# lanxinger/spz

Hardware: AMD Instinct MI355X
Metric: Gaussians/s encode+decode (SH3, 10M pts) (higher is better)
Workload: dtype f32

## Files before the change

### spz_amd/csrc/spz_abi.hip

```cpp
#include <hip/hip_runtime.h>

#include <cmath>
#include <cstdint>
#include <algorithm>
#include <cstdlib>
#include <cstring>
#include <mutex>

#include "spz_amd.h"
#include "spz_common.hpp"
#include "spz_kernel_params.hpp"

namespace spz_amd_detail {
thread_local int g_last_hip_error = 0;

}

namespace {

using namespace spz_amd_detail;

constexpr uint32_t kMagic = 0x5053474eu;

unsigned long long sh_elem_mask_ext(uint32_t sh15, int sh_dim) {
// ... 85 lines not shown
    SPZ_HIP_TRY(hipMalloc(reinterpret_cast<void **>(&d), sizeof(float) * kTableFloats));
    hipError_t e = hipMemcpy(d, g_tables.host, sizeof(float) * kTableFloats, hipMemcpyHostToDevice);
    if (e != hipSuccess) {
      g_last_hip_error = (int)e;
      (void)hipFree(d);
      return SPZ_AMD_ERR_HIP;
    }
    g_tables.dev[device] = d;
  }
  *dev_tables = g_tables.dev[device];
  return SPZ_AMD_OK;
}
}

namespace {

int grid_for(int device, uint32_t total_tiles, uint32_t *grid) {
  uint32_t cap = 0x7fffffffu;
  if (kMaxBlocksPerCU > 0) {
    static int cus[kMaxDevices] = {0};
    if (cus[device] == 0) {
      int n = 0;
      SPZ_HIP_TRY(hipDeviceGetAttribute(&n, hipDeviceAttributeMultiprocessorCount, device));
      cus[device] = (n > 0) ? n : 256;
    }
    cap = (uint32_t)cus[device] * (uint32_t)kMaxBlocksPerCU;
  }
  uint32_t g = total_tiles < cap ? total_tiles : cap;
#if SPZ_XCD_REMAP
  g = ((total_tiles + 7u) / 8u) * 8u;
#endif
  *grid = g > 0 ? g : 1;
  return SPZ_AMD_OK;
}

void add_section(KParams *p, uint32_t tile_units, uint32_t kind, uint8_t *bytes, float *floats,
                 unsigned long long n_elems) {
  if (n_elems == 0) return;
  SecDesc &s = p->sec[p->n_sec++];
  s.bytes = bytes;
  s.floats = floats;
  s.n_elems = n_elems;
  s.n_units = (n_elems + 3) / 4;
  s.tile_begin = p->total_tiles;
  s.tile_skip = 0;
  s.kind = kind;
  p->total_tiles += (uint32_t)((s.n_units + tile_units - 1) / tile_units);
}

void interleave_sections(KParams *p) {
  const uint32_t n = p->n_sec, total = p->total_tiles;
  if (n < 2 || total < 4 * kIlPeriod) return;
  constexpr uint32_t G = SPZ_IL_GROUP;
  uint32_t tiles[SPZ_AMD_NUM_SECTIONS], count[SPZ_AMD_NUM_SECTIONS], used = 0;
  uint32_t big = 0, part_total = 0;
  for (uint32_t k = 0; k < n; ++k) {
    tiles[k] = (k + 1 < n ? p->sec[k + 1].tile_begin : total) - p->sec[k].tile_begin;
    big = tiles[k] > tiles[big] ? k : big;
  }
  auto takes_part = [&](uint32_t k) {
    return !SPZ_IL_ONLY_ROT || k == big || p->sec[k].kind == KIND_ROT_S3 || p->sec[k].kind == KIND_ROT_F3;
  };
  for (uint32_t k = 0; k < n; ++k) part_total += takes_part(k) ? tiles[k] : 0u;
  for (uint32_t k = 0; k < n; ++k) {
    count[k] = takes_part(k) ? (uint32_t)(((unsigned long long)tiles[k] * kIlPeriod + part_total / 2) / part_total) : 0u;
    used += count[k];
  }
  if (used > kIlPeriod && count[big] <= used - kIlPeriod) return;
  count[big] = count[big] + kIlPeriod - used;
  uint32_t reps = 0xffffffffu;
  for (uint32_t k = 0; k < n; ++k) {
    if (count[k]) reps = tiles[k] / (count[k] * G) < reps ? tiles[k] / (count[k] * G) : reps;
  }
  if (reps == 0 || reps == 0xffffffffu) return;
  uint32_t given[SPZ_AMD_NUM_SECTIONS] = {};
  for (uint32_t slot = 0; slot < kIlPeriod; ++slot) {
    uint32_t best = n;
    unsigned long long best_pos = ~0ull;
    for (uint32_t k = 0; k < n; ++k) {
      if (given[k] >= count[k]) continue;
      const unsigned long long pos = (2ull * given[k] + 1ull) * kIlPeriod * 1024ull / (2ull * count[k]);
      if (pos < best_pos) {
        best_pos = pos;
        best = k;
      }
    }
    p->il_sec[slot] = (uint8_t)best;
    p->il_rank[slot] = (uint8_t)given[best];
    ++given[best];
  }
  p->il_tiles = reps * kIlPeriod * G;
  uint32_t begin = p->il_tiles;
  for (uint32_t k = 0; k < n; ++k) {
    p->il_count[k] = (uint8_t)count[k];
    p->sec[k].tile_skip = reps * count[k] * G;
    p->sec[k].tile_begin = begin;
    begin += tiles[k] - reps * count[k] * G;
  }
}

int grid_order_override() {
  const char *e = std::getenv("SPZ_AMD_GRID_ORDER");
  if (e == nullptr) return 0;
  if (std::strcmp(e, "sequential") == 0) return 1;
  if (std::strcmp(e, "interleaved") == 0) return 2;
  return 0;
}

int layout_impl(uint64_t n, int sh_degree, int version, spz_amd_layout *out) {
  const int sd = sh_dim_for_degree(sh_degree);
  if (sd < 0 || version < 1 || version > 3 || out == nullptr) return SPZ_AMD_ERR_INVALID_ARG;
  const uint32_t bpp[SPZ_AMD_NUM_SECTIONS] = {version == 1 ? 6u : 9u, 1u, 3u, 3u, version >= 3 ? 4u : 3u,
                                               (uint32_t)sd * 3u};
  uint64_t off = 16;
  for (int s = 0; s < SPZ_AMD_NUM_SECTIONS; ++s) {
    out->bytes_per_point[s] = bpp[s];
    out->offset[s] = off;
    out->bytes[s] = n * bpp[s];
    off += out->bytes[s];
  }
  out->total_bytes = off;
  return SPZ_AMD_OK;
}

int encode_impl(const spz_amd_cloud_in *cl, uint64_t first, uint64_t count, uint64_t n_total, int sh_degree,
                int antialiased, int from_coord, int version, int write_header, uint8_t *d_stream,
                size_t capacity, void *hip_stream, unsigned section_mask = 0x3fu) {
  if (cl == nullptr || d_stream == nullptr || !valid_coord(from_coord)) return SPZ_AMD_ERR_INVALID_ARG;
  if (version == 1) return SPZ_AMD_ERR_UNSUPPORTED;
  spz_amd_layout lay;
  int rc = layout_impl(n_total, sh_degree, version, &lay);
  if (rc != SPZ_AMD_OK) return rc;
  if (n_total > 0xffffffffull || first > n_total || count > n_total - first) return SPZ_AMD_ERR_INVALID_ARG;
  if (capacity < lay.total_bytes) return SPZ_AMD_ERR_CAPACITY;
  const int sd = sh_dim_for_degree(sh_degree);
  if (count > 0 && (!cl->positions || !cl->scales || !cl->rotations || !cl->alphas || !cl->colors ||
                    (sd > 0 && !cl->sh))) {
    return SPZ_AMD_ERR_INVALID_ARG;
  }
  int device = 0;
  rc = current_device(&device);
  if (rc != SPZ_AMD_OK) return rc;
  KParams p = {};
  rc = ensure_tables(device, &p.tables);
  if (rc != SPZ_AMD_OK) return rc;

  const FlipMasks fm = flip_masks(from_coord, SPZ_AMD_RUB);
  p.flip_p = fm.p;
  p.flip_q = fm.q;
  p.sh_mask_ext = sh_elem_mask_ext(fm.sh15, sd);
  p.sh_d = (uint32_t)sd * 3u;
  p.pos_scale = 0.0f;
  auto frag = [&](int s) { return d_stream + lay.offset[s] + first * lay.bytes_per_point[s]; };
  auto fl = [](const float *q) { return const_cast<float *>(q); };
  auto want = [&](int s) { return ((section_mask >> s) & 1u) != 0u; };
  if (want(SPZ_AMD_SEC_SH)) add_section(&p, EncGeom::kTileUnits, KIND_SH, frag(SPZ_AMD_SEC_SH), fl(cl->sh), count * (uint64_t)sd * 3u);
  if (want(SPZ_AMD_SEC_POSITIONS)) add_section(&p, EncGeom::kTileUnits, KIND_POS24, frag(SPZ_AMD_SEC_POSITIONS), fl(cl->positions), count * 3u);
  if (want(SPZ_AMD_SEC_ROTATIONS)) {
    add_section(&p, EncGeom::kTileUnits, version >= 3 ? KIND_ROT_S3 : KIND_ROT_F3, frag(SPZ_AMD_SEC_ROTATIONS), fl(cl->rotations),
                count * 4u);
  }
  if (want(SPZ_AMD_SEC_SCALES)) add_section(&p, EncGeom::kTileUnits, KIND_SCALE, frag(SPZ_AMD_SEC_SCALES), fl(cl->scales), count * 3u);
  if (want(SPZ_AMD_SEC_COLORS)) add_section(&p, EncGeom::kTileUnits, KIND_COLOR, frag(SPZ_AMD_SEC_COLORS), fl(cl->colors), count * 3u);
  if (want(SPZ_AMD_SEC_ALPHAS)) add_section(&p, EncGeom::kTileUnits, KIND_ALPHA, frag(SPZ_AMD_SEC_ALPHAS), fl(cl->alphas), count);
  if (write_header) {
    p.header_dst = d_stream;
    p.header_words[0] = kMagic;
    p.header_words[1] = (uint32_t)version;
    p.header_words[2] = (uint32_t)n_total;
    p.header_words[3] = (uint32_t)sh_degree | (12u << 8) | ((antialiased ? 1u : 0u) << 16);
  }
  if (p.total_tiles == 0 && !write_header) return SPZ_AMD_OK;
  {
    const int order = grid_order_override();
    if (order == 2 || (order == 0 && (SPZ_ENC_INTERLEAVE == 1 || (SPZ_ENC_INTERLEAVE == 2 && sd == 0)))) interleave_sections(&p);
  }
  uint32_t grid = 1;
  rc = grid_for(device, p.total_tiles, &grid);
  if (rc != SPZ_AMD_OK) return rc;
  hipLaunchKernelGGL(spz_encode_kernel, dim3(grid), dim3(EncGeom::kBlock), 0, static_cast<hipStream_t>(hip_stream), p);
  SPZ_HIP_TRY(hipGetLastError());
  return SPZ_AMD_OK;
}

int check_header_fields(const spz_amd_header *h) {
  if (h == nullptr) return SPZ_AMD_ERR_INVALID_ARG;
  if (h->version < 1 || h->version > 3) return SPZ_AMD_ERR_VERSION;
  if (h->sh_degree > 3) return SPZ_AMD_ERR_SH_DEGREE;
  return SPZ_AMD_OK;
}

int decode_impl(const uint8_t *d_stream, size_t size, const spz_amd_header *hdr, uint64_t first, uint64_t count,
                int to_coord, const spz_amd_cloud_out *cl, void *hip_stream) {
  if (d_stream == nullptr || cl == nullptr || !valid_coord(to_coord)) return SPZ_AMD_ERR_INVALID_ARG;
  int rc = check_header_fields(hdr);
  if (rc != SPZ_AMD_OK) return rc;
  const uint64_t n_total = hdr->num_points;
  if (first > n_total || count > n_total - first) return SPZ_AMD_ERR_INVALID_ARG;
  spz_amd_layout lay;
  rc = layout_impl(n_total, hdr->sh_degree, (int)hdr->version, &lay);
  if (rc != SPZ_AMD_OK) return rc;
  if (size < lay.total_bytes) return SPZ_AMD_ERR_SHORT_STREAM;
  const int sd = sh_dim_for_degree(hdr->sh_degree);
  if (count > 0 && (!cl->positions || !cl->scales || !cl->rotations || !cl->alphas || !cl->colors ||
                    (sd > 0 && !cl->sh))) {
    return SPZ_AMD_ERR_INVALID_ARG;
  }
  if (count == 0) return SPZ_AMD_OK;
  int device = 0;
// ... 250 lines not shown
  p.out_positions = cl->positions;
  p.out_scales = cl->scales;
  p.out_rotations = cl->rotations;
  p.out_alphas = cl->alphas;
  p.out_colors = cl->colors;
  p.out_sh = cl->sh;
  p.indices = d_indices;
  p.count = count;
  p.num_points = hdr->num_points;
  p.version = hdr->version;
  p.sh_dim = (uint32_t)sd;
  const FlipMasks fm = flip_masks(SPZ_AMD_RUB, to_coord);
  p.flip_p = fm.p;
  p.flip_q = fm.q;
  p.flip_sh15 = fm.sh15;
  p.sh_elem_mask = sh_elem_mask_ext(fm.sh15, sd);
  p.pos_scale = (float)(1.0 / (double)(int32_t)(1u << (hdr->fractional_bits & 31)));
  const unsigned long long items = count * (unsigned long long)(sd > 0 ? sd * 3 : 3);
  unsigned long long blocks = (items + 255) / 256;
  if (blocks > 65536ull * 16) blocks = 65536ull * 16;
  hipLaunchKernelGGL(spz_decode_gather_kernel, dim3((unsigned)blocks), dim3(256), 0, static_cast<hipStream_t>(hip_stream), p);
  SPZ_HIP_TRY(hipGetLastError());
  return SPZ_AMD_OK;
}

int spz_amd_convert_coordinates_device(float *d_positions, float *d_rotations, float *d_sh, uint64_t num_points,
                                       int sh_degree, int from_coord, int to_coord, void *hip_stream) {
  const int sd = sh_dim_for_degree(sh_degree);
  if (sd < 0 || !valid_coord(from_coord) || !valid_coord(to_coord)) return SPZ_AMD_ERR_INVALID_ARG;
  if (num_points == 0) return SPZ_AMD_OK;
  int device = 0;
  int rc = current_device(&device);
  if (rc != SPZ_AMD_OK) return rc;
  KParams p = {};
  const FlipMasks fm = flip_masks(from_coord, to_coord);
  p.flip_p = fm.p;
  p.flip_q = fm.q;
  p.sh_mask_ext = sh_elem_mask_ext(fm.sh15, sd);
  p.sh_d = (uint32_t)sd * 3u;
  if (d_sh) add_section(&p, FlipGeom::kTileUnits, KIND_FLIP_SH, nullptr, d_sh, num_points * (uint64_t)sd * 3u);
  if (d_positions) add_section(&p, FlipGeom::kTileUnits, KIND_FLIP_POS, nullptr, d_positions, num_points * 3u);
  if (d_rotations) add_section(&p, FlipGeom::kTileUnits, KIND_FLIP_ROT, nullptr, d_rotations, num_points * 4u);
  if (p.total_tiles == 0) return SPZ_AMD_OK;
  uint32_t grid = 1;
  rc = grid_for(device, p.total_tiles, &grid);
  if (rc != SPZ_AMD_OK) return rc;
  hipLaunchKernelGGL(spz_flip_kernel, dim3(grid), dim3(FlipGeom::kBlock), 0, static_cast<hipStream_t>(hip_stream), p);
  SPZ_HIP_TRY(hipGetLastError());
  return SPZ_AMD_OK;
}


int spz_amd_selftest_device(int mode, uint64_t begin, uint64_t count, uint64_t result[3], void *hip_stream) {
  if (result == nullptr || mode < 0 || mode > (int)SELFTEST_UNPACK_S3) return SPZ_AMD_ERR_INVALID_ARG;
  int device = 0;
  int rc = current_device(&device);
  if (rc != SPZ_AMD_OK) return rc;
  hipStream_t st = static_cast<hipStream_t>(hip_stream);
  unsigned long long *d = nullptr;
  SPZ_HIP_TRY(hipMalloc(reinterpret_cast<void **>(&d), 3 * sizeof(unsigned long long)));
  const unsigned long long init[3] = {0ull, ~0ull, 0ull};
  hipError_t e = hipMemcpyAsync(d, init, sizeof(init), hipMemcpyHostToDevice, st);
  if (e == hipSuccess && count > 0) {
    SelfTestParams p = {(uint32_t)mode, begin, count, d};
    unsigned long long blocks = (count + 255) / 256;
    if (blocks > 256ull * 64) blocks = 256ull * 64;
    hipLaunchKernelGGL(spz_selftest_kernel, dim3((unsigned)blocks), dim3(256), 0, st, p);
    e = hipGetLastError();
  }
  unsigned long long out[3] = {0, 0, 0};
  if (e == hipSuccess) e = hipMemcpyAsync(out, d, sizeof(out), hipMemcpyDeviceToHost, st);
  if (e == hipSuccess) e = hipStreamSynchronize(st);
  (void)hipFree(d);
  if (e != hipSuccess) {
    g_last_hip_error = (int)e;
    return SPZ_AMD_ERR_HIP;
  }
  for (int i = 0; i < 3; ++i) result[i] = out[i];
  return SPZ_AMD_OK;
}

int spz_amd_get_tables(float alpha_decode[256], float color_decode[256], float alpha_thresholds[255]) {
  std::lock_guard<std::mutex> lock(g_tables_mutex);
  if (!g_tables.host_ready) build_host_tables();
  if (alpha_decode) std::memcpy(alpha_decode, g_tables.host + kTableAlphaDec, 256 * sizeof(float));
  if (color_decode) std::memcpy(color_decode, g_tables.host + kTableColorDec, 256 * sizeof(float));
  if (alpha_thresholds) std::memcpy(alpha_thresholds, g_tables.host + kTableAlphaThr, 255 * sizeof(float));
  return SPZ_AMD_OK;
}

}
```

### spz_amd/csrc/spz_kernel_params.hpp

```cpp
#pragma once

#include <hip/hip_runtime.h>

#include <cstdint>

#include "spz_amd.h"

namespace spz_amd_detail {

#ifndef SPZ_DEC_BLOCK
#define SPZ_DEC_BLOCK 256
#endif
#ifndef SPZ_DEC_UNROLL
#define SPZ_DEC_UNROLL 4
#endif
#ifndef SPZ_DEC_WC
#define SPZ_DEC_WC 0
#endif
#ifndef SPZ_DEC_NTL
#define SPZ_DEC_NTL 1
#endif
#ifndef SPZ_DEC_NTS
#define SPZ_DEC_NTS 1
#endif
#ifndef SPZ_ENC_BLOCK
#define SPZ_ENC_BLOCK 256
#endif
#ifndef SPZ_ENC_UNROLL
#define SPZ_ENC_UNROLL 4
#endif
#ifndef SPZ_ENC_WC
#define SPZ_ENC_WC 1
#endif
#ifndef SPZ_ENC_NTL
#define SPZ_ENC_NTL 1
#endif
#ifndef SPZ_ENC_NTS
#define SPZ_ENC_NTS 0
#endif
#ifndef SPZ_ENC_MIN_WAVES
#define SPZ_ENC_MIN_WAVES 6
#endif
#ifndef SPZ_ENC_SCHED_BARRIER
#define SPZ_ENC_SCHED_BARRIER 1
#endif
#ifndef SPZ_DEC_REVERSE
#define SPZ_DEC_REVERSE 0
#endif
#ifndef SPZ_DEC_HOT_MIB
#define SPZ_DEC_HOT_MIB 0
#endif
#ifndef SPZ_XCD_REMAP
#define SPZ_XCD_REMAP 0
#endif
#ifndef SPZ_ENC_INTERLEAVE
#define SPZ_ENC_INTERLEAVE 2
#endif
#ifndef SPZ_DEC_INTERLEAVE
#define SPZ_DEC_INTERLEAVE 2
#endif
#ifndef SPZ_IL_GROUP
#define SPZ_IL_GROUP 8
#endif
#ifndef SPZ_IL_ONLY_ROT
#define SPZ_IL_ONLY_ROT 0
#endif
#ifndef SPZ_QUAT_FAST
#define SPZ_QUAT_FAST 1
#endif
#ifndef SPZ_BLOCKS_PER_CU
#define SPZ_BLOCKS_PER_CU 0
#endif

template <int BLOCK_, int UNROLL_, bool WC_, bool NTL_, bool NTS_>
struct Geom {
  static constexpr int kBlock = BLOCK_;
  static constexpr int kUnroll = UNROLL_;
  static constexpr int kTileUnits = BLOCK_ * UNROLL_;
  static constexpr bool kWaveContig = WC_;
  static constexpr bool kNtLoad = NTL_;
  static constexpr bool kNtStore = NTS_;
  __device__ static __forceinline__ uint32_t local_unit(int r, uint32_t tid) {
    if constexpr (WC_) return ((tid >> 6) * (uint32_t)UNROLL_ + (uint32_t)r) * 64u + (tid & 63u);
    else return (uint32_t)(r * BLOCK_) + tid;
  }
};
using DecGeom = Geom<SPZ_DEC_BLOCK, SPZ_DEC_UNROLL, SPZ_DEC_WC != 0, SPZ_DEC_NTL != 0, SPZ_DEC_NTS != 0>;
using DecGeomHot = Geom<SPZ_DEC_BLOCK, SPZ_DEC_UNROLL, SPZ_DEC_WC != 0, false, SPZ_DEC_NTS != 0>;
using EncGeom = Geom<SPZ_ENC_BLOCK, SPZ_ENC_UNROLL, SPZ_ENC_WC != 0, SPZ_ENC_NTL != 0, SPZ_ENC_NTS != 0>;
using FlipGeom = Geom<256, 4, false, false, false>;
constexpr int kMaxBlocksPerCU = SPZ_BLOCKS_PER_CU;

enum SecKind : uint32_t {
  KIND_POS24 = 0,
  KIND_POS16,
  KIND_ALPHA,
  KIND_COLOR,
  KIND_SCALE,
  KIND_ROT_S3,
  KIND_ROT_F3,
  KIND_SH,
  KIND_FLIP_POS,
  KIND_FLIP_ROT,
  KIND_FLIP_SH,
};

struct SecDesc {
  uint8_t *bytes;
  float *floats;
  unsigned long long n_elems;
  unsigned long long n_units;
  uint32_t tile_begin;
  uint32_t tile_skip;
  uint32_t kind;
};

constexpr uint32_t kIlPeriod = 61;

struct KParams {
  SecDesc sec[SPZ_AMD_NUM_SECTIONS];
  uint32_t n_sec;
  uint32_t total_tiles;
  uint32_t flip_p;
  uint32_t flip_q;
  unsigned long long sh_mask_ext;
  uint32_t sh_d;
  float pos_scale;
  const float *tables;
  uint8_t *header_dst;
  uint32_t header_words[4];
  uint32_t plain_tiles;
  uint32_t il_tiles;
  uint8_t il_count[8];
  uint8_t il_sec[64];
  uint8_t il_rank[64];
};

constexpr int kTableAlphaDec = 0;
constexpr int kTableColorDec = 256;
constexpr int kTableAlphaThr = 512;
constexpr int kTableFloats = 768;

struct GatherParams {
  const uint8_t *positions, *alphas, *colors, *scales, *rotations, *sh;
  float *out_positions, *out_scales, *out_rotations, *out_alphas, *out_colors, *out_sh;
  const uint32_t *indices;
  unsigned long long count;
  uint32_t num_points;
  uint32_t version;
  uint32_t sh_dim;
  uint32_t flip_p, flip_q, flip_sh15;
  unsigned long long sh_elem_mask;
  float pos_scale;
  const float *tables;
};

enum SelfTestMode : uint32_t {
  SELFTEST_DIV_SQRT1_2 = 0,
  SELFTEST_DIV_511 = 1,
  SELFTEST_SQRT = 2,
  SELFTEST_QUOTIENT = 3,
  SELFTEST_PACK_S3 = 4,
  SELFTEST_PACK_F3 = 5,
  SELFTEST_UNPACK_S3 = 6,
};
struct SelfTestParams {
  uint32_t mode;
  unsigned long long begin, count;
  unsigned long long *mismatches;
};

int ensure_tables(int device, const float **dev_tables);

__global__ void spz_selftest_kernel(const SelfTestParams p);
__global__ void spz_decode_gather_kernel(const GatherParams p);
__global__ void spz_decode_kernel(const KParams p);
__global__ void spz_encode_kernel(const KParams p);
__global__ void spz_flip_kernel(const KParams p);

}
```

### spz_amd/csrc/spz_kernels.hip

```cpp
#include <hip/hip_runtime.h>

#include <cstdint>

#include "spz_amd.h"
#include "spz_common.hpp"
#include "spz_kernel_params.hpp"
#include "spz_quant.hpp"

#pragma clang fp contract(off)

namespace spz_amd_detail {
namespace {

struct __attribute__((packed, aligned(1))) U32x1 { uint32_t a; };
struct __attribute__((packed, aligned(1))) U32x2 { uint32_t a, b; };
struct __attribute__((packed, aligned(1))) U32x3 { uint32_t a, b, c; };
struct __attribute__((packed, aligned(1))) U8x3 { uint8_t a, b, c; };

struct Raw3 { uint32_t a, b, c; };

typedef float v4f_t __attribute__((ext_vector_type(4)));
typedef v4f_t v4f_a4 __attribute__((aligned(4)));
typedef uint32_t u32_a1 __attribute__((aligned(1)));

// ... 163 lines not shown
  const uint32_t pb = tile_phase_base<KIND, D, G>(tile_local);
  if (base + G::kTileUnits <= full_units) {
    Raw3 raw[G::kUnroll];
#pragma unroll
    for (int r = 0; r < G::kUnroll; ++r) raw[r] = load_raw<KIND, G>(src, base + G::local_unit(r, tid));
#pragma unroll
    for (int r = 0; r < G::kUnroll; ++r) {
      const uint32_t local = G::local_unit(r, tid);
      store_f4<G::kNtStore>(dst, base + local, decode_unit<KIND, D>(raw[r], unit_phase<KIND, D>(pb, local), c));
    }
  } else {
#pragma unroll
    for (int r = 0; r < G::kUnroll; ++r) {
      const uint32_t local = G::local_unit(r, tid);
      const unsigned long long u = base + local;
      if (u < full_units) {
        store_f4<G::kNtStore>(dst, u, decode_unit<KIND, D>(load_raw<KIND, G>(src, u), unit_phase<KIND, D>(pb, local), c));
      } else if (u < s.n_units) {
        if constexpr (KIND != KIND_ROT_S3 && KIND != KIND_ROT_F3) {
          const uint32_t m = (uint32_t)(s.n_elems - u * 4ull);
          F32x4 v = decode_unit<KIND, D>(load_raw_partial<KIND>(src, u, m), unit_phase<KIND, D>(pb, local), c);
          float *p = dst + u * 4ull;
          p[0] = v.x;
          if (m > 1) p[1] = v.y;
          if (m > 2) p[2] = v.z;
        }
      }
    }
  }
}

template <int KIND, class G>
__device__ __forceinline__ void decode_tile_sh_dispatch(const SecDesc &s, uint32_t tile_local, const DecodeCtx &c,
                                                        uint32_t sh_d) {
  if (sh_d == 45u) decode_tile<KIND, 45, G>(s, tile_local, c);
  else if (sh_d == 24u) decode_tile<KIND, 24, G>(s, tile_local, c);
  else decode_tile<KIND, 9, G>(s, tile_local, c);
}

__device__ __forceinline__ uint32_t first_tile(const KParams &p) {
#if SPZ_XCD_REMAP
  const uint32_t chunk = (p.total_tiles + 7u) / 8u;
  const uint32_t t = (blockIdx.x & 7u) * chunk + (blockIdx.x >> 3);
  return ((blockIdx.x >> 3) < chunk && t < p.total_tiles) ? t : 0xffffffffu;
#else
  (void)p;
  return blockIdx.x;
#endif
}

__device__ __forceinline__ uint32_t find_section(const KParams &p, uint32_t tile) {
  uint32_t si = 0;
#pragma unroll
  for (uint32_t k = 1; k < SPZ_AMD_NUM_SECTIONS; ++k) {
    if (k < p.n_sec && tile >= p.sec[k].tile_begin) si = k;
  }
  return si;
}

struct TileRef { uint32_t si, tl; };
__device__ __forceinline__ TileRef locate_tile(const KParams &p, uint32_t tile) {
  TileRef t;
  if (tile < p.il_tiles) {
    const uint32_t group = tile / (uint32_t)SPZ_IL_GROUP, within = tile % (uint32_t)SPZ_IL_GROUP;
    const uint32_t rep = group / kIlPeriod, k = group - rep * kIlPeriod;
    t.si = p.il_sec[k];
    t.tl = (rep * p.il_count[t.si] + p.il_rank[k]) * (uint32_t)SPZ_IL_GROUP + within;
  } else {
    t.si = find_section(p, tile);
    t.tl = tile - p.sec[t.si].tile_begin + p.sec[t.si].tile_skip;
  }
  return t;
}

template <class G>
__device__ __forceinline__ void stage_tables(float *lut, const float *__restrict__ tables) {
  for (uint32_t i = threadIdx.x; i < kTableFloats; i += G::kBlock) lut[i] = tables[i];
  __syncthreads();
}

}

template <class G>
__device__ __forceinline__ void decode_one_tile(const KParams &p, const SecDesc &s, uint32_t tl, const DecodeCtx &c,
                                                float *lut, bool &lut_ready) {
  switch (s.kind) {
    case KIND_POS24: decode_tile<KIND_POS24, 0, G>(s, tl, c); break;
    case KIND_POS16: decode_tile<KIND_POS16, 0, G>(s, tl, c); break;
    case KIND_ALPHA:
    case KIND_COLOR:
      if (!lut_ready) {
        stage_tables<G>(lut, p.tables);
        lut_ready = true;
      }
      if (s.kind == KIND_ALPHA) decode_tile<KIND_ALPHA, 0, G>(s, tl, c);
      else decode_tile<KIND_COLOR, 0, G>(s, tl, c);
      break;
    case KIND_SCALE: decode_tile<KIND_SCALE, 0, G>(s, tl, c); break;
    case KIND_ROT_S3: decode_tile<KIND_ROT_S3, 0, G>(s, tl, c); break;
    case KIND_ROT_F3: decode_tile<KIND_ROT_F3, 0, G>(s, tl, c); break;
    case KIND_SH: decode_tile_sh_dispatch<KIND_SH, G>(s, tl, c, p.sh_d); break;
    default: break;
  }
}

__global__ __launch_bounds__(DecGeom::kBlock) void spz_decode_kernel(const KParams p) {
  __shared__ float lut[kTableFloats];
// ... 4 lines not shown
  c.sh_mask_ext = p.sh_mask_ext;
  c.pos_scale = p.pos_scale;
  c.lut = lut;
  for (uint32_t t0 = first_tile(p); t0 < p.total_tiles; t0 = SPZ_XCD_REMAP ? 0xffffffffu : t0 + gridDim.x) {
    const uint32_t tile = SPZ_DEC_REVERSE ? p.total_tiles - 1u - t0 : t0;
    const TileRef ref = locate_tile(p, tile);
    const SecDesc &s = p.sec[ref.si];
    const uint32_t tl = ref.tl;
    if (SPZ_DEC_REVERSE && SPZ_DEC_NTL && t0 < p.plain_tiles) decode_one_tile<DecGeomHot>(p, s, tl, c, lut, lut_ready);
    else decode_one_tile<DecGeom>(p, s, tl, c, lut, lut_ready);
  }
}

namespace {

struct EncodeCtx {
  uint32_t flip_p, flip_q;
  unsigned long long sh_mask_ext;
  const float *lut;
};

template <int KIND, int D>
__device__ __forceinline__ Raw3 encode_unit(F32x4 v, uint32_t phase, const EncodeCtx &c) {
  Raw3 o = {0u, 0u, 0u};
  if constexpr (KIND == KIND_POS24) {
    uint32_t sb = pos_sign_bits(c.flip_p, phase);
    uint32_t f0 = (uint32_t)position_fixed(xor_sign(v.x, sb & 1u), 4096.0f) & 0xffffffu;
    uint32_t f1 = (uint32_t)position_fixed(xor_sign(v.y, (sb >> 1) & 1u), 4096.0f) & 0xffffffu;
    uint32_t f2 = (uint32_t)position_fixed(xor_sign(v.z, (sb >> 2) & 1u), 4096.0f) & 0xffffffu;
    uint32_t f3 = (uint32_t)position_fixed(xor_sign(v.w, (sb >> 3) & 1u), 4096.0f) & 0xffffffu;
    o.a = f0 | (f1 << 24);
    o.b = (f1 >> 8) | (f2 << 16);
    o.c = (f2 >> 16) | (f3 << 8);
  } else if constexpr (KIND == KIND_ALPHA) {
    const float *t = c.lut + kTableAlphaThr;
    o.a = alpha_byte(v.x, t) | (alpha_byte(v.y, t) << 8) | (alpha_byte(v.z, t) << 16) | (alpha_byte(v.w, t) << 24);
  } else if constexpr (KIND == KIND_COLOR) {
    constexpr float k = 0.15f * 255.0f;
    constexpr float h = 0.5f * 255.0f;
    o.a = pack_u8x4(to_uint8_f(fmul_sep(v.x, k) + h), to_uint8_f(fmul_sep(v.y, k) + h),
                    to_uint8_f(fmul_sep(v.z, k) + h), to_uint8_f(fmul_sep(v.w, k) + h));
  } else if constexpr (KIND == KIND_SCALE) {
    o.a = pack_u8x4(scale_to_byte_f(v.x), scale_to_byte_f(v.y), scale_to_byte_f(v.z), scale_to_byte_f(v.w));
  } else if constexpr (KIND == KIND_ROT_S3) {
    o.a = pack_quat_smallest_three(v, c.flip_q);
  } else if constexpr (KIND == KIND_ROT_F3) {
    o.a = pack_quat_first_three(v, c.flip_q);
  } else {
    uint32_t sb = (uint32_t)(c.sh_mask_ext >> phase) & 0xfu;
    uint32_t j0 = phase, j1 = phase + 1, j2 = phase + 2, j3 = phase + 3;
    j1 -= (j1 >= (uint32_t)D) ? (uint32_t)D : 0u;
    j2 -= (j2 >= (uint32_t)D) ? (uint32_t)D : 0u;
    j3 -= (j3 >= (uint32_t)D) ? (uint32_t)D : 0u;
    o.a = pack_u8x4(quantize_sh_f(xor_sign(v.x, sb & 1u), j0 < 9u), quantize_sh_f(xor_sign(v.y, (sb >> 1) & 1u), j1 < 9u),
                    quantize_sh_f(xor_sign(v.z, (sb >> 2) & 1u), j2 < 9u), quantize_sh_f(xor_sign(v.w, (sb >> 3) & 1u), j3 < 9u));
  }
  return o;
}

template <int KIND, class G>
__device__ __forceinline__ void store_raw(uint8_t *__restrict__ dst, unsigned long long u, Raw3 r) {
  if constexpr (KIND == KIND_POS24) {
    if constexpr (G::kNtStore) {
      uint8_t *q = dst + u * 12ull;
      st_u32<true>(q, r.a); st_u32<true>(q + 4, r.b); st_u32<true>(q + 8, r.c);
    } else {
      U32x3 t;
      t.a = r.a; t.b = r.b; t.c = r.c;
      *reinterpret_cast<U32x3 *>(dst + u * 12ull) = t;
    }
  } else if constexpr (KIND == KIND_ROT_F3) {
    U8x3 t;
    t.a = (uint8_t)r.a; t.b = (uint8_t)(r.a >> 8); t.c = (uint8_t)(r.a >> 16);
    *reinterpret_cast<U8x3 *>(dst + u * 3ull) = t;
  } else {
    st_u32<G::kNtStore>(dst + u * 4ull, r.a);
  }
}

template <int KIND, int D, class G>
__device__ __forceinline__ void encode_tile(const SecDesc &s, uint32_t tile_local, const EncodeCtx &c) {
  const unsigned long long base = (unsigned long long)tile_local * G::kTileUnits;
  const uint32_t tid = threadIdx.x;
  const float *__restrict__ src = s.floats;
  uint8_t *__restrict__ dst = s.bytes;
  const unsigned long long full_units = s.n_elems >> 2;
  const uint32_t pb = tile_phase_base<KIND, D, G>(tile_local);
  if (base + G::kTileUnits <= full_units) {
    F32x4 v[G::kUnroll];
#pragma unroll
    for (int r = 0; r < G::kUnroll; ++r) v[r] = load_f4<G::kNtLoad>(src, base + G::local_unit(r, tid));
#pragma unroll
    for (int r = 0; r < G::kUnroll; ++r) {
      const uint32_t local = G::local_unit(r, tid);
      store_raw<KIND, G>(dst, base + local, encode_unit<KIND, D>(v[r], unit_phase<KIND, D>(pb, local), c));
#if SPZ_ENC_SCHED_BARRIER
      __builtin_amdgcn_sched_barrier(0);
#endif
    }
  } else {
#pragma unroll
    for (int r = 0; r < G::kUnroll; ++r) {
      const uint32_t local = G::local_unit(r, tid);
      const unsigned long long u = base + local;
      if (u < full_units) {
        store_raw<KIND, G>(dst, u, encode_unit<KIND, D>(load_f4<G::kNtLoad>(src, u), unit_phase<KIND, D>(pb, local), c));
      } else if (u < s.n_units) {
        if constexpr (KIND != KIND_ROT_S3 && KIND != KIND_ROT_F3) {
          const uint32_t m = (uint32_t)(s.n_elems - u * 4ull);
          const float *p = src + u * 4ull;
          F32x4 v;
          v.x = p[0];
          v.y = (m > 1) ? p[1] : 0.0f;
          v.z = (m > 2) ? p[2] : 0.0f;
          v.w = 0.0f;
          Raw3 r3 = encode_unit<KIND, D>(v, unit_phase<KIND, D>(pb, local), c);
          constexpr uint32_t bpe = (KIND == KIND_POS24) ? 3u : 1u;
          uint8_t *q = dst + u * (4ull * bpe);
          const uint32_t w[3] = {r3.a, r3.b, r3.c};
          for (uint32_t i = 0; i < m * bpe; ++i) q[i] = (uint8_t)(w[i >> 2] >> ((i & 3u) * 8u));
        }
      }
    }
  }
}

template <int KIND>
__device__ __forceinline__ void encode_tile_sh_dispatch(const SecDesc &s, uint32_t tile_local, const EncodeCtx &c,
                                                        uint32_t sh_d) {
  if (sh_d == 45u) encode_tile<KIND, 45, EncGeom>(s, tile_local, c);
  else if (sh_d == 24u) encode_tile<KIND, 24, EncGeom>(s, tile_local, c);
  else encode_tile<KIND, 9, EncGeom>(s, tile_local, c);
}

}

__global__ __launch_bounds__(EncGeom::kBlock, SPZ_ENC_MIN_WAVES) void spz_encode_kernel(const KParams p) {
  __shared__ float lut[kTableFloats];
  bool lut_ready = false;
  EncodeCtx c;
  c.flip_p = p.flip_p;
  c.flip_q = p.flip_q;
  c.sh_mask_ext = p.sh_mask_ext;
  c.lut = lut;
  if (blockIdx.x == 0 && threadIdx.x < 16 && p.header_dst != nullptr) {
    p.header_dst[threadIdx.x] = (uint8_t)(p.header_words[threadIdx.x >> 2] >> ((threadIdx.x & 3u) * 8u));
  }
  for (uint32_t tile = first_tile(p); tile < p.total_tiles; tile = SPZ_XCD_REMAP ? 0xffffffffu : tile + gridDim.x) {
    const TileRef ref = locate_tile(p, tile);
    const SecDesc &s = p.sec[ref.si];
    const uint32_t tl = ref.tl;
    switch (s.kind) {
      case KIND_POS24: encode_tile<KIND_POS24, 0, EncGeom>(s, tl, c); break;
      case KIND_ALPHA:
        if (!lut_ready) {
          stage_tables<EncGeom>(lut, p.tables);
          lut_ready = true;
        }
        encode_tile<KIND_ALPHA, 0, EncGeom>(s, tl, c);
        break;
      case KIND_COLOR: encode_tile<KIND_COLOR, 0, EncGeom>(s, tl, c); break;
      case KIND_SCALE: encode_tile<KIND_SCALE, 0, EncGeom>(s, tl, c); break;
      case KIND_ROT_S3: encode_tile<KIND_ROT_S3, 0, EncGeom>(s, tl, c); break;
      case KIND_ROT_F3: encode_tile<KIND_ROT_F3, 0, EncGeom>(s, tl, c); break;
      case KIND_SH: encode_tile_sh_dispatch<KIND_SH>(s, tl, c, p.sh_d); break;
      default: break;
    }
  }
}

namespace {

template <int KIND, int D>
__device__ __forceinline__ F32x4 flip_unit(F32x4 v, uint32_t phase, const KParams &p) {
  uint32_t sb;
  if constexpr (KIND == KIND_FLIP_POS) sb = pos_sign_bits(p.flip_p, phase);
  else if constexpr (KIND == KIND_FLIP_ROT) sb = p.flip_q & 7u;
  else sb = (uint32_t)(p.sh_mask_ext >> phase) & 0xfu;
  F32x4 o;
  o.x = mul_pm1(v.x, sb & 1u);
  o.y = mul_pm1(v.y, (sb >> 1) & 1u);
  o.z = mul_pm1(v.z, (sb >> 2) & 1u);
  o.w = (KIND == KIND_FLIP_ROT) ? v.w : mul_pm1(v.w, (sb >> 3) & 1u);
  return o;
}

template <int KIND, int D>
__device__ __forceinline__ void flip_tile(const SecDesc &s, uint32_t tile_local, const KParams &p) {
  const unsigned long long base = (unsigned long long)tile_local * FlipGeom::kTileUnits;
  const uint32_t tid = threadIdx.x;
  float *buf = s.floats;
  const unsigned long long full_units = s.n_elems >> 2;
  const uint32_t pb = tile_phase_base<KIND, D, FlipGeom>(tile_local);
#pragma unroll
  for (int r = 0; r < FlipGeom::kUnroll; ++r) {
    const uint32_t local = FlipGeom::local_unit(r, tid);
    const unsigned long long u = base + local;
    const uint32_t ph = unit_phase<KIND, D>(pb, local);
    if (u < full_units) {
      store_f4<false>(buf, u, flip_unit<KIND, D>(load_f4<false>(buf, u), ph, p));
    } else if (u < s.n_units) {
      const uint32_t m = (uint32_t)(s.n_elems - u * 4ull);
      float *q = buf + u * 4ull;
      F32x4 v;
      v.x = q[0];
      v.y = (m > 1) ? q[1] : 0.0f;
      v.z = (m > 2) ? q[2] : 0.0f;
      v.w = 0.0f;
      F32x4 o = flip_unit<KIND, D>(v, ph, p);
      q[0] = o.x;
      if (m > 1) q[1] = o.y;
      if (m > 2) q[2] = o.z;
    }
  }
}

}

// ... 125 lines not shown

}

__global__ __launch_bounds__(256) void spz_selftest_kernel(const SelfTestParams p) {
  const unsigned long long stride = (unsigned long long)gridDim.x * blockDim.x;
  unsigned long long bad = 0, first = ~0ull, seen = 0;
  for (unsigned long long k = (unsigned long long)blockIdx.x * blockDim.x + threadIdx.x; k < p.count; k += stride) {
    const unsigned long long i = p.begin + k;
    bool differs = false, used = true;
    if (p.mode == SELFTEST_DIV_SQRT1_2 || p.mode == SELFTEST_DIV_511) {
      const float x = __uint_as_float((uint32_t)i);
      used = i <= 0x7f800000ull && (i == 0ull || (x >= 0x1p-100f && x <= 0x1p126f));
      if (used) {
        float fast, plain;
        if (p.mode == SELFTEST_DIV_SQRT1_2) {
          fast = div_by_const(x, kSqrt1_2, kRcpSqrt1_2);
          plain = x / kSqrt1_2;
        } else {
          fast = div_by_const(x, 511.0f, kRcp511);
          plain = x / 511.0f;
        }
        differs = __float_as_uint(fast) != __float_as_uint(plain);
      }
    } else if (p.mode == SELFTEST_SQRT) {
      const float x = __uint_as_float((uint32_t)i);
      used = i <= 0x7f800000ull && x >= 0x1p-80f && x <= 0x1p82f;
      if (used) differs = __float_as_uint(sqrt_cr(x)) != __float_as_uint(__builtin_sqrtf(x));
    } else if (p.mode == SELFTEST_QUOTIENT) {
      const unsigned long long h = mix64(i);
      const uint32_t eb = 87u + (uint32_t)(h & 0xffu) % 82u;
      const float b = __uint_as_float((eb << 23) | (uint32_t)((h >> 8) & 0x7fffffu));
      uint32_t ea = eb + 1u - (uint32_t)((h >> 31) & 0xffu) % (eb + 2u - 87u);
      float a = __uint_as_float((ea << 23) | (uint32_t)((h >> 40) & 0x7fffffu));
      if ((i & 1ull) != 0ull) a = __uint_as_float((__float_as_uint(b) & ~0xfu) | (uint32_t)((h >> 60) & 0xfu));
      if (a > 2.0f * b) a = b;
      const float fast = quat_quotient(a, b, refined_rcp(b));
      const float plain = a / b;
      differs = __float_as_uint(fast) != __float_as_uint(plain);
    } else if (p.mode == SELFTEST_PACK_S3 || p.mode == SELFTEST_PACK_F3) {
      const F32x4 r = window_quat(i);
      const uint32_t flip_q = (uint32_t)(mix64(~i) & 7u);
      used = quat_fast_ok(r);
      if (used) {
        const Quat4 qf = normalized_flipped_fast(r, flip_q), qg = normalized_flipped(r, flip_q);
        differs = __float_as_uint(qf.q0) != __float_as_uint(qg.q0) || __float_as_uint(qf.q1) != __float_as_uint(qg.q1) ||
                  __float_as_uint(qf.q2) != __float_as_uint(qg.q2) || __float_as_uint(qf.q3) != __float_as_uint(qg.q3);
        if (p.mode == SELFTEST_PACK_S3) differs = differs || smallest_three_fields_fast(qf) != smallest_three_fields(qg);
      }
    } else if (p.mode == SELFTEST_UNPACK_S3) {
      const uint32_t flip_q = (uint32_t)(i >> 32) & 7u;
      const F32x4 f = unpack_quat_smallest_three_t<true>((uint32_t)i, flip_q), g = unpack_quat_smallest_three_t<false>((uint32_t)i, flip_q);
      differs = __float_as_uint(f.x) != __float_as_uint(g.x) || __float_as_uint(f.y) != __float_as_uint(g.y) ||
                __float_as_uint(f.z) != __float_as_uint(g.z) || __float_as_uint(f.w) != __float_as_uint(g.w);
    } else {
      used = false;
    }
    seen += used ? 1ull : 0ull;
    if (differs) {
      ++bad;
      first = i < first ? i : first;
    }
  }
  for (int off = 32; off >= 1; off >>= 1) {
    bad += __shfl_down(bad, off);
    seen += __shfl_down(seen, off);
    const unsigned long long o = __shfl_down(first, off);
    first = o < first ? o : first;
  }
  if ((threadIdx.x & 63u) == 0u) {
    if (bad) atomicAdd(&p.mismatches[0], bad);
    if (first != ~0ull) atomicMin(&p.mismatches[1], first);
    atomicAdd(&p.mismatches[2], seen);
  }
}

}
```

### spz_amd/csrc/spz_quant.hpp

```cpp
#pragma once

#include <hip/hip_runtime.h>

#include <cstdint>

#include "spz_common.hpp"
#include "spz_kernel_params.hpp"

#pragma clang fp contract(off)

namespace spz_amd_detail {
namespace {

__device__ __forceinline__ float fmul_sep(float a, float b) {
  float r = a * b;
  asm volatile("" : "+v"(r));
  return r;
}
__device__ __forceinline__ float fadd_sep(float a, float b) {
  float r = a + b;
  asm volatile("" : "+v"(r));
  return r;
}

__device__ __forceinline__ float round_half_away(float x) {
  float t = __builtin_truncf(x);
  float d = __builtin_fabsf(x - t);
  float one = __builtin_copysignf(1.0f, x);
  return (d >= 0.5f) ? (t + one) : t;
}

__device__ __forceinline__ int32_t cvt_i32_x86(float r) {
  return (r >= -2147483648.0f && r < 2147483648.0f) ? (int32_t)r : (int32_t)0x80000000;
}

__device__ __forceinline__ uint32_t cvt_u32_x86(float r) {
  if (r > -9223372036854775808.0f && r < 9223372036854775808.0f) {
    return (uint32_t)(long long)r;
  }
  return 0u;
}

__device__ __forceinline__ float to_uint8_f(float x) {
  float r = round_half_away(x);
  return __builtin_fminf(__builtin_fmaxf(r, 0.0f), 255.0f);
}
__device__ __forceinline__ uint32_t to_uint8(float x) { return (uint32_t)to_uint8_f(x); }

__device__ __forceinline__ float quantize_sh_f(float x, bool degree1) {
  const float inv_b = degree1 ? 0.125f : 0.0625f;
  const float b = degree1 ? 8.0f : 16.0f;
  float r = round_half_away(x * 128.0f);
  float k = __builtin_floorf(__builtin_fmaf(r, inv_b, 0.5f));
  float v = __builtin_fminf(__builtin_fmaxf(__builtin_fmaf(k, b, 128.0f), 0.0f), 255.0f);
  return (r < 2147483520.0f) ? v : 0.0f;
}

__device__ __forceinline__ uint32_t pack_u8x4(float a, float b, float c, float d) {
  uint32_t w = __builtin_amdgcn_cvt_pk_u8_f32(a, 0u, 0u);
  w = __builtin_amdgcn_cvt_pk_u8_f32(b, 1u, w);
  w = __builtin_amdgcn_cvt_pk_u8_f32(c, 2u, w);
  return __builtin_amdgcn_cvt_pk_u8_f32(d, 3u, w);
}

__device__ __forceinline__ float scale_from_byte(uint32_t b) { return (float)b / 16.0f - 10.0f; }
__device__ __forceinline__ float scale_to_byte_f(float v) { return to_uint8_f(fadd_sep(v, 10.0f) * 16.0f); }
__device__ __forceinline__ float sh_from_byte(uint32_t b) { return ((float)b - 128.0f) / 128.0f; }
__device__ __forceinline__ int32_t position_fixed(float v, float scale) { return cvt_i32_x86(round_half_away(v * scale)); }

constexpr float kSqrt1_2 = (float)0.707106781186547524401;

constexpr uint32_t kFastLoBits = 0x2b800000u;
constexpr uint32_t kFastHiBits = 0x53800000u;

__device__ __forceinline__ bool quat_fast_ok(F32x4 r) {
  const uint32_t a0 = __float_as_uint(r.x) & 0x7fffffffu, a1 = __float_as_uint(r.y) & 0x7fffffffu;
  const uint32_t a2 = __float_as_uint(r.z) & 0x7fffffffu, a3 = __float_as_uint(r.w) & 0x7fffffffu;
  const uint32_t lo = min(min(a0 - 1u, a1 - 1u), min(a2 - 1u, a3 - 1u));
  const uint32_t hi = max(max(a0, a1), max(a2, a3));
  return lo >= kFastLoBits - 1u && hi <= kFastHiBits && hi != 0u;
}

__device__ __forceinline__ float sqrt_cr(float x) {
  const float s = __builtin_amdgcn_sqrtf(x);
  const float dn = __uint_as_float(__float_as_uint(s) - 1u);
  const float up = __uint_as_float(__float_as_uint(s) + 1u);
  const float r_dn = __builtin_fmaf(-dn, s, x);
  const float r_up = __builtin_fmaf(-up, s, x);
  float o = (r_dn <= 0.0f) ? dn : s;
  o = (r_up > 0.0f) ? up : o;
  return o;
}

__device__ __forceinline__ float refined_rcp(float b) {
  const float y0 = __builtin_amdgcn_rcpf(b);
  const float e = __builtin_fmaf(-b, y0, 1.0f);
  return __builtin_fmaf(e, y0, y0);
}

__device__ __forceinline__ float quat_quotient(float a, float b, float y) {
  const float m = a * y;
  const float r0 = __builtin_fmaf(-b, m, a);
  const float q1 = __builtin_fmaf(r0, y, m);
  const float r1 = __builtin_fmaf(-b, q1, a);
  return __builtin_fmaf(r1, y, q1);
}

__device__ __forceinline__ float div_by_const(float x, float c, float rc) {
  const float m = x * rc;
// ... 157 lines not shown
```

Measured before the change: 10.39 billion.

## Simplify SH quantization math and add optional row-grouped SH encode path

After: 10.34 billion (median of 2 runs). About the same (-0.5%).

```diff
diff --git a/spz_amd/csrc/spz_abi.hip b/spz_amd/csrc/spz_abi.hip
--- a/spz_amd/csrc/spz_abi.hip
+++ b/spz_amd/csrc/spz_abi.hip
@@ -161,7 +161,7 @@
   const uint32_t n = p->n_sec, total = p->total_tiles;
   if (n < 2 || total < 4 * kIlPeriod) return;
   constexpr uint32_t G = SPZ_IL_GROUP;
-  uint32_t tiles[SPZ_AMD_NUM_SECTIONS], count[SPZ_AMD_NUM_SECTIONS], used = 0;
+  uint32_t tiles[kMaxSec], count[kMaxSec], used = 0;
   uint32_t big = 0, part_total = 0;
   for (uint32_t k = 0; k < n; ++k) {
     tiles[k] = (k + 1 < n ? p->sec[k + 1].tile_begin : total) - p->sec[k].tile_begin;
@@ -182,7 +182,7 @@
     if (count[k]) reps = tiles[k] / (count[k] * G) < reps ? tiles[k] / (count[k] * G) : reps;
   }
   if (reps == 0 || reps == 0xffffffffu) return;
-  uint32_t given[SPZ_AMD_NUM_SECTIONS] = {};
+  uint32_t given[kMaxSec] = {};
   for (uint32_t slot = 0; slot < kIlPeriod; ++slot) {
     uint32_t best = n;
     unsigned long long best_pos = ~0ull;
@@ -263,7 +263,17 @@
   auto frag = [&](int s) { return d_stream + lay.offset[s] + first * lay.bytes_per_point[s]; };
   auto fl = [](const float *q) { return const_cast<float *>(q); };
   auto want = [&](int s) { return ((section_mask >> s) & 1u) != 0u; };
-  if (want(SPZ_AMD_SEC_SH)) add_section(&p, EncGeom::kTileUnits, KIND_SH, frag(SPZ_AMD_SEC_SH), fl(cl->sh), count * (uint64_t)sd * 3u);
+  if (want(SPZ_AMD_SEC_SH) && sd > 0) {
+    const uint64_t d = (uint64_t)sd * 3u;
+    uint64_t rows_points = 0;
+    if (SPZ_ENC_SH_ROWS && EncGeom::kBlock == 256) {
+      const uint64_t run = (uint64_t)kShRowsGroupPoints * kShRowsR;
+      rows_points = count / run * run;
+    }
+    add_section(&p, 256u * kShRowsR, KIND_SH_ROWS, frag(SPZ_AMD_SEC_SH), fl(cl->sh), rows_points * d);
+    add_section(&p, EncGeom::kTileUnits, KIND_SH, frag(SPZ_AMD_SEC_SH) + rows_points * d,
+                cl->sh ? fl(cl->sh) + rows_points * d : nullptr, (count - rows_points) * d);
+  }
   if (want(SPZ_AMD_SEC_POSITIONS)) add_section(&p, EncGeom::kTileUnits, KIND_POS24, frag(SPZ_AMD_SEC_POSITIONS), fl(cl->positions), count * 3u);
   if (want(SPZ_AMD_SEC_ROTATIONS)) {
     add_section(&p, EncGeom::kTileUnits, version >= 3 ? KIND_ROT_S3 : KIND_ROT_F3, frag(SPZ_AMD_SEC_ROTATIONS), fl(cl->rotations),
@@ -620,7 +630,7 @@
 
 
 int spz_amd_selftest_device(int mode, uint64_t begin, uint64_t count, uint64_t result[3], void *hip_stream) {
-  if (result == nullptr || mode < 0 || mode > (int)SELFTEST_UNPACK_S3) return SPZ_AMD_ERR_INVALID_ARG;
+  if (result == nullptr || mode < 0 || mode > (int)SELFTEST_SH_QUANT) return SPZ_AMD_ERR_INVALID_ARG;
   int device = 0;
   int rc = current_device(&device);
   if (rc != SPZ_AMD_OK) return rc;
diff --git a/spz_amd/csrc/spz_kernel_params.hpp b/spz_amd/csrc/spz_kernel_params.hpp
--- a/spz_amd/csrc/spz_kernel_params.hpp
+++ b/spz_amd/csrc/spz_kernel_params.hpp
@@ -71,6 +71,12 @@
 #ifndef SPZ_BLOCKS_PER_CU
 #define SPZ_BLOCKS_PER_CU 0
 #endif
+#ifndef SPZ_ENC_SH_ROWS
+#define SPZ_ENC_SH_ROWS 0
+#endif
+#ifndef SPZ_ENC_SH_ROWS_R
+#define SPZ_ENC_SH_ROWS_R 4
+#endif
 
 template <int BLOCK_, int UNROLL_, bool WC_, bool NTL_, bool NTS_>
 struct Geom {
@@ -103,7 +109,12 @@
   KIND_FLIP_POS,
   KIND_FLIP_ROT,
   KIND_FLIP_SH,
+  KIND_SH_ROWS,
 };
+constexpr uint32_t kShRowsR = SPZ_ENC_SH_ROWS_R;
+constexpr uint32_t kShRowsGroupPoints = 1024;
+
+constexpr uint32_t kMaxSec = SPZ_AMD_NUM_SECTIONS + 1;
 
 struct SecDesc {
   uint8_t *bytes;
@@ -118,7 +129,7 @@
 constexpr uint32_t kIlPeriod = 61;
 
 struct KParams {
-  SecDesc sec[SPZ_AMD_NUM_SECTIONS];
+  SecDesc sec[kMaxSec];
   uint32_t n_sec;
   uint32_t total_tiles;
   uint32_t flip_p;
@@ -163,6 +174,7 @@
   SELFTEST_PACK_S3 = 4,
   SELFTEST_PACK_F3 = 5,
   SELFTEST_UNPACK_S3 = 6,
+  SELFTEST_SH_QUANT = 7,
 };
 struct SelfTestParams {
   uint32_t mode;
diff --git a/spz_amd/csrc/spz_kernels.hip b/spz_amd/csrc/spz_kernels.hip
--- a/spz_amd/csrc/spz_kernels.hip
+++ b/spz_amd/csrc/spz_kernels.hip
@@ -239,7 +239,7 @@
 __device__ __forceinline__ uint32_t find_section(const KParams &p, uint32_t tile) {
   uint32_t si = 0;
 #pragma unroll
-  for (uint32_t k = 1; k < SPZ_AMD_NUM_SECTIONS; ++k) {
+  for (uint32_t k = 1; k < kMaxSec; ++k) {
     if (k < p.n_sec && tile >= p.sec[k].tile_begin) si = k;
   }
   return si;
@@ -350,10 +350,43 @@
     j1 -= (j1 >= (uint32_t)D) ? (uint32_t)D : 0u;
     j2 -= (j2 >= (uint32_t)D) ? (uint32_t)D : 0u;
     j3 -= (j3 >= (uint32_t)D) ? (uint32_t)D : 0u;
-    o.a = pack_u8x4(quantize_sh_f(xor_sign(v.x, sb & 1u), j0 < 9u), quantize_sh_f(xor_sign(v.y, (sb >> 1) & 1u), j1 < 9u),
-                    quantize_sh_f(xor_sign(v.z, (sb >> 2) & 1u), j2 < 9u), quantize_sh_f(xor_sign(v.w, (sb >> 3) & 1u), j3 < 9u));
+    o.a = pack_u8x4(quantize_sh_class(v.x, sb << 31, sh_class(j0 < 9u)), quantize_sh_class(v.y, (sb >> 1) << 31, sh_class(j1 < 9u)),
+                    quantize_sh_class(v.z, (sb >> 2) << 31, sh_class(j2 < 9u)), quantize_sh_class(v.w, (sb >> 3) << 31, sh_class(j3 < 9u)));
   }
   return o;
+}
+
+template <int D, class G>
+__device__ __forceinline__ void encode_tile_sh_rows(const SecDesc &s, uint32_t tile_local, const EncodeCtx &c) {
+  constexpr uint32_t kGroupUnits = (uint32_t)D * 256u;
+  const uint32_t grp = tile_local / (uint32_t)D, rho = tile_local - grp * (uint32_t)D;
+  uint32_t tid = threadIdx.x;
+  asm volatile("" : "+v"(tid));
+  const uint32_t lu = rho * 256u + tid;
+  const uint32_t phase = (4u * lu) % (uint32_t)D;
+  const uint32_t sb = (uint32_t)(c.sh_mask_ext >> phase) & 0xfu;
+  uint32_t j1 = phase + 1, j2 = phase + 2, j3 = phase + 3;
+  j1 -= (j1 >= (uint32_t)D) ? (uint32_t)D : 0u;
+  j2 -= (j2 >= (uint32_t)D) ? (uint32_t)D : 0u;
+  j3 -= (j3 >= (uint32_t)D) ? (uint32_t)D : 0u;
+  const uint32_t f0 = sb << 31, f1 = (sb >> 1) << 31, f2 = (sb >> 2) << 31, f3 = (sb >> 3) << 31;
+  const ShClass q0 = sh_class(phase < 9u), q1 = sh_class(j1 < 9u), q2 = sh_class(j2 < 9u), q3 = sh_class(j3 < 9u);
+  const unsigned long long u0 = (unsigned long long)grp * (kShRowsR * kGroupUnits) + lu;
+  if (u0 + (unsigned long long)(kShRowsR - 1u) * kGroupUnits >= s.n_units) return;
+  const float *__restrict__ src = s.floats;
+  uint8_t *__restrict__ dst = s.bytes;
+  F32x4 v[kShRowsR];
+#pragma unroll
+  for (uint32_t r = 0; r < kShRowsR; ++r) v[r] = load_f4<G::kNtLoad>(src, u0 + (unsigned long long)r * kGroupUnits);
+#pragma unroll
+  for (uint32_t r = 0; r < kShRowsR; ++r) {
+    const uint32_t w = pack_u8x4(quantize_sh_class(v[r].x, f0, q0), quantize_sh_class(v[r].y, f1, q1),
+                                 quantize_sh_class(v[r].z, f2, q2), quantize_sh_class(v[r].w, f3, q3));
+    st_u32<G::kNtStore>(dst + (u0 + (unsigned long long)r * kGroupUnits) * 4ull, w);
+#if SPZ_ENC_SCHED_BARRIER
+    __builtin_amdgcn_sched_barrier(0);
+#endif
+  }
 }
 
 template <int KIND, class G>
@@ -379,7 +412,8 @@
 template <int KIND, int D, class G>
 __device__ __forceinline__ void encode_tile(const SecDesc &s, uint32_t tile_local, const EncodeCtx &c) {
   const unsigned long long base = (unsigned long long)tile_local * G::kTileUnits;
-  const uint32_t tid = threadIdx.x;
+  uint32_t tid = threadIdx.x;
+  asm volatile("" : "+v"(tid));
   const float *__restrict__ src = s.floats;
   uint8_t *__restrict__ dst = s.bytes;
   const unsigned long long full_units = s.n_elems >> 2;
@@ -462,6 +496,13 @@
       case KIND_ROT_S3: encode_tile<KIND_ROT_S3, 0, EncGeom>(s, tl, c); break;
       case KIND_ROT_F3: encode_tile<KIND_ROT_F3, 0, EncGeom>(s, tl, c); break;
       case KIND_SH: encode_tile_sh_dispatch<KIND_SH>(s, tl, c, p.sh_d); break;
+#if SPZ_ENC_SH_ROWS
+      case KIND_SH_ROWS:
+        if (p.sh_d == 45u) encode_tile_sh_rows<45, EncGeom>(s, tl, c);
+        else if (p.sh_d == 24u) encode_tile_sh_rows<24, EncGeom>(s, tl, c);
+        else encode_tile_sh_rows<9, EncGeom>(s, tl, c);
+        break;
+#endif
       default: break;
     }
   }
@@ -693,6 +734,15 @@
       const F32x4 f = unpack_quat_smallest_three_t<true>((uint32_t)i, flip_q), g = unpack_quat_smallest_three_t<false>((uint32_t)i, flip_q);
       differs = __float_as_uint(f.x) != __float_as_uint(g.x) || __float_as_uint(f.y) != __float_as_uint(g.y) ||
                 __float_as_uint(f.z) != __float_as_uint(g.z) || __float_as_uint(f.w) != __float_as_uint(g.w);
+    } else if (p.mode == SELFTEST_SH_QUANT) {
+      const float x = __uint_as_float((uint32_t)i);
+      const bool degree1 = ((i >> 32) & 1ull) == 0ull;
+      const uint32_t flip = (uint32_t)((i >> 33) & 1ull);
+      used = i < (1ull << 34);
+      if (used) {
+        differs = __float_as_uint(quantize_sh_class(x, flip << 31, sh_class(degree1))) !=
+                  __float_as_uint(quantize_sh_ref_f(xor_sign(x, flip), degree1));
+      }
     } else {
       used = false;
     }
diff --git a/spz_amd/csrc/spz_quant.hpp b/spz_amd/csrc/spz_quant.hpp
--- a/spz_amd/csrc/spz_quant.hpp
+++ b/spz_amd/csrc/spz_quant.hpp
@@ -47,7 +47,7 @@
 }
 __device__ __forceinline__ uint32_t to_uint8(float x) { return (uint32_t)to_uint8_f(x); }
 
-__device__ __forceinline__ float quantize_sh_f(float x, bool degree1) {
+__device__ __forceinline__ float quantize_sh_ref_f(float x, bool degree1) {
   const float inv_b = degree1 ? 0.125f : 0.0625f;
   const float b = degree1 ? 8.0f : 16.0f;
   float r = round_half_away(x * 128.0f);
@@ -55,6 +55,28 @@
   float v = __builtin_fminf(__builtin_fmaxf(__builtin_fmaf(k, b, 128.0f), 0.0f), 255.0f);
   return (r < 2147483520.0f) ? v : 0.0f;
 }
+
+struct ShClass {
+  float g, c, b;
+};
+__device__ __forceinline__ ShClass sh_class(bool degree1) {
+  ShClass k;
+  k.g = degree1 ? 16.0f : 8.0f;
+  k.c = degree1 ? 0.0625f : 0.03125f;
+  k.b = degree1 ? 8.0f : 16.0f;
+  return k;
+}
+__device__ __forceinline__ float quantize_sh_class(float x, uint32_t flip, ShClass q) {
+  const float z = __uint_as_float(__float_as_uint(x) ^ flip);
+  const float t = __builtin_fabsf(z) * q.g;
+  const float ft = __builtin_floorf(t);
+  const float fr = t - ft;
+  const float thr = 0.5f - __builtin_copysignf(q.c, z);
+  const float k = ft + ((fr >= thr) ? 1.0f : 0.0f);
+  const float v = __builtin_fminf(__builtin_fmaxf(__builtin_fmaf(k, __builtin_copysignf(q.b, z), 128.0f), 0.0f), 255.0f);
+  return (z < 16777215.0f) ? v : 0.0f;
+}
+__device__ __forceinline__ float quantize_sh_f(float x, bool degree1) { return quantize_sh_class(x, 0u, sh_class(degree1)); }
 
 __device__ __forceinline__ uint32_t pack_u8x4(float a, float b, float c, float d) {
   uint32_t w = __builtin_amdgcn_cvt_pk_u8_f32(a, 0u, 0u);
```
